# yj-yu/Recurrent_Gaze_Prediction

Measured on AMD Instinct MI355X. Metric: frames/sec (49x49 saliency maps), gaze_grcn 16-frame clips, higher is better.
Workload: dtype bf16; 1 GPU; gaze_grcn end-to-end: synthetic 16x112x112x3 windows -> C3D conv1a-5b -> 1024->512 proj -> ConvGRU(512->128, 7x7) -> deconv head -> 49x49 softmax maps; clips_per_gpu=64, n_lstm_steps=16, parallelism=dp1 (clip-sharded replicas, no collective), weights=random init (reference initialisers), GRU filters std 0.05

## Files before the change

include/rgp.h:

```cpp
#ifndef RGP_H_
#define RGP_H_
#include <stddef.h>

#ifdef __cplusplus
extern "C" {
#endif

#define RGP_OK 0
#define RGP_EINVAL (-1)
#define RGP_EHIP (-2)
#define RGP_EWORKSPACE (-3)
#define RGP_ESTATE (-4)
#define RGP_ETIMEOUT (-5)

#define RGP_F32 0
#define RGP_BF16 1

typedef void* rgp_stream_t;

const char* rgp_last_error(void);
int rgp_version(void);
int rgp_device_arch(char* buf, int buflen);

typedef struct rgp_grcn rgp_grcn_t;
// ... 204 lines not shown
int rgp_shallownet_forward(rgp_shallownet_t* plan, const float* frames, int n_frames, float* saliency,
                           float* saliency7, rgp_stream_t stream);

int rgp_shallownet_create_ex(rgp_shallownet_t** plan, int max_frames, int image_hw, int dtype, int save_for_backward);
int rgp_shallownet_backward(rgp_shallownet_t* plan, int n_frames, const float* d_saliency, const rgp_shallownet_weights* grads,
                            rgp_stream_t stream);

typedef struct rgp_cascade rgp_cascade_t;

typedef struct rgp_cascade_weights {
  const float *proj_c3d_W, *proj_c3d_b;
  const float *bottom_Wz, *bottom_Uz, *bottom_Wr, *bottom_Ur, *bottom_W, *bottom_U;
  const float* upsampling_weight;
  const float *top_Wz, *top_Uz, *top_Wr, *top_Ur, *top_W, *top_U;
  const float *fc1_w, *fc1_b, *fc2_w, *fc2_b;
  rgp_shallownet_weights shallownet;
} rgp_cascade_weights;

int rgp_cascade_create(rgp_cascade_t** plan, int batch, int n_steps, int image_hw, int dtype);
int rgp_cascade_destroy(rgp_cascade_t* plan);
size_t rgp_cascade_workspace_bytes(const rgp_cascade_t* plan);
int rgp_cascade_bind_workspace(rgp_cascade_t* plan, void* workspace, size_t bytes, rgp_stream_t stream);
int rgp_cascade_set_weights(rgp_cascade_t* plan, const rgp_cascade_weights* w, rgp_stream_t stream);
int rgp_cascade_forward(rgp_cascade_t* plan, const float* frame_images, const float* c3d_input, float* gazemaps,
                        rgp_stream_t stream);
int rgp_cascade_create_ex(rgp_cascade_t** plan, int batch, int n_steps, int image_hw, int dtype, int save_for_backward);
int rgp_cascade_backward(rgp_cascade_t* plan, const float* gazemaps, const float* gt_gazemap, const rgp_cascade_weights* grads,
                         float* d_rows, rgp_stream_t stream);
int rgp_cascade_set_dropout(rgp_cascade_t* plan, float keep_prob, const unsigned char* mask);
int rgp_cascade_read_buffer(rgp_cascade_t* plan, const char* name, float* dst, rgp_stream_t stream);

typedef struct rgp_c3d rgp_c3d_t;

typedef struct rgp_c3d_weights {
  const float* w[8];
  const float* b[8];
} rgp_c3d_weights;

int rgp_c3d_create(rgp_c3d_t** plan, int max_windows, int dtype);
int rgp_c3d_destroy(rgp_c3d_t* plan);
size_t rgp_c3d_workspace_bytes(const rgp_c3d_t* plan);
int rgp_c3d_bind_workspace(rgp_c3d_t* plan, void* workspace, size_t bytes, rgp_stream_t stream);
int rgp_c3d_set_weights(rgp_c3d_t* plan, const rgp_c3d_weights* w, rgp_stream_t stream);
int rgp_c3d_forward(rgp_c3d_t* plan, const float* video, int n_windows, float* features, void* rows,
                    rgp_stream_t stream);
int rgp_c3d_forward_frames(rgp_c3d_t* plan, const unsigned char* frames, int n_frames, int frame_h, int frame_w,
                           const int* window_starts, int n_windows, const float* mean_cube, float* features, void* rows,
                           rgp_stream_t stream);
int rgp_c3d_frames_to_video(rgp_c3d_t* plan, const unsigned char* frames, int n_frames, int frame_h, int frame_w,
                            const int* window_starts, int n_windows, const float* mean_cube, float* video,
                            rgp_stream_t stream);
int rgp_c3d_read_layer(rgp_c3d_t* plan, int layer, int n_windows, float* dst, rgp_stream_t stream);
size_t rgp_c3d_layer_elems(const rgp_c3d_t* plan, int layer, int n_windows);

int rgp_c3d_create_ex(rgp_c3d_t** plan, int max_windows, int dtype, int flags);
#define RGP_C3D_SAVE_FOR_BACKWARD 1
#define RGP_C3D_KERNELS_IGEMM 2
#define RGP_C3D_KERNELS_TILE128 4
#define RGP_C3D_CONV2A_ROWWISE 8
const char* rgp_c3d_layer_kernel_name(const rgp_c3d_t* plan, int layer, int n_windows);
size_t rgp_c3d_param_elems(const rgp_c3d_t* plan);
size_t rgp_c3d_param_offset(const rgp_c3d_t* plan, int layer, int is_bias);
int rgp_c3d_backward(rgp_c3d_t* plan, const float* d_features, const float* d_rows, int n_windows, float* grads,
                     rgp_stream_t stream);
int rgp_c3d_wait_layer_grads(rgp_c3d_t* plan, int layer, rgp_stream_t waiting_stream);
int rgp_c3d_read_grad_image(rgp_c3d_t* plan, int layer, int n_windows, float* dst, rgp_stream_t stream);

#define RGP_C3D_STAGES 9
int rgp_c3d_profile_enable(rgp_c3d_t* plan, int enable);
int rgp_c3d_profile_read(rgp_c3d_t* plan, double ms[RGP_C3D_STAGES], long long calls[RGP_C3D_STAGES]);

#define RGP_METRICS_MAX_PIX 4096
#define RGP_METRICS_MAX_FIX 256
#define RGP_METRICS_MAX_THRESHOLDS 1024
#define RGP_METRICS_COUNT 6
#define RGP_METRIC_SIM 1
#define RGP_METRIC_CC 2
#define RGP_METRIC_AUC_JUDD 4
#define RGP_METRIC_AUC_BORJI 8
#define RGP_METRIC_AUC_SHUFFLED 16
#define RGP_METRIC_NSS 32
#define RGP_METRIC_ALL 63
#define RGP_METRIC_ROW_SIM 0
#define RGP_METRIC_ROW_CC 1
#define RGP_METRIC_ROW_AUC_JUDD 2
#define RGP_METRIC_ROW_AUC_BORJI 3
#define RGP_METRIC_ROW_AUC_SHUFFLED 4
#define RGP_METRIC_ROW_NSS 5
#define RGP_METRICS_DEVICE_DRAWS 1
#define RGP_METRICS_NO_JITTER 2
#define RGP_METRICS_PRED_F64 4
#define RGP_METRICS_GT_F64 8

typedef struct rgp_metrics_args {
  const void* pred;
  const void* gt;
  const float* fix;
  const float* other;
  long long other_stride;
  int n_frames, height, width;
  unsigned metrics;
  unsigned flags;
  int n_rep;
  int neg_stride;
  double step_size;
  const double* judd_jitter;
// ... 65 lines not shown
```

recurrent_gaze_prediction_amd/_lib.py:

```python
import ctypes
import os

import torch

LIB_PATH = os.path.join(os.path.dirname(os.path.abspath(__file__)), 'librgp_hip.so')

RGP_F32, RGP_BF16 = 0, 1
RGP_ETIMEOUT = -5
RGP_GRCN_SAVE_FOR_BACKWARD, RGP_GRCN_PER_STEP, RGP_GRCN_UNFOLDED_HEAD = 1, 2, 4
RGP_C3D_SAVE_FOR_BACKWARD, RGP_C3D_KERNELS_IGEMM, RGP_C3D_KERNELS_TILE128, RGP_C3D_CONV2A_ROWWISE = 1, 2, 4, 8
RGP_C3DCONV_SAVE_FOR_BACKWARD, RGP_C3DCONV_STAGED, RGP_C3DCONV_FUSED = 1, 2, 4
RGP_LSTM_SAVE_FOR_BACKWARD, RGP_LSTM_PER_STEP, RGP_LSTM_PERSISTENT, RGP_LSTM_BPTT_PERSISTENT = 1, 2, 4, 8
RGP_GRCN77_SAVE_FOR_BACKWARD, RGP_GRCN77_PER_STEP = 1, 2
RGP_FAULT_SEQ_LOST_MEMBER, RGP_FAULT_BPTT_LOST_MEMBER = 1, 2
RGP_ACTION_NN, RGP_ACTION_SVM = 0, 1
RGP_ACTION_USE_GAZEMAP, RGP_ACTION_SAVE_FOR_BACKWARD, RGP_ACTION_UNFUSED = 1, 2, 4
RGP_GRCN_GRADS_TOP, RGP_GRCN_GRADS_GRU, RGP_GRCN_GRADS_PROJ = 0, 1, 2
RGP_SQNORM_PARTIALS = 256
RGP_METRICS_MAX_PIX, RGP_METRICS_MAX_FIX, RGP_METRICS_MAX_THRESHOLDS, RGP_METRICS_COUNT = 4096, 256, 1024, 6
METRIC_BITS = {'sim': 1, 'cc': 2, 'AUC_Judd': 4, 'AUC_Borji': 8, 'AUC_shuffled': 16, 'NSS': 32}
METRIC_ROWS = {'sim': 0, 'cc': 1, 'AUC_Judd': 2, 'AUC_Borji': 3, 'AUC_shuffled': 4, 'NSS': 5}
RGP_METRICS_DEVICE_DRAWS, RGP_METRICS_NO_JITTER, RGP_METRICS_PRED_F64, RGP_METRICS_GT_F64 = 1, 2, 4, 8
RGP_GTMAPS_MAX_PIX, RGP_GTMAPS_MAX_OBSERVERS, RGP_GTMAPS_MAX_RADIUS = 4096, 32, 32
DTYPES = {'f32': RGP_F32, 'fp32': RGP_F32, 'float32': RGP_F32, 'bf16': RGP_BF16, 'bfloat16': RGP_BF16}
# ... 133 lines not shown
    'rgp_lstm_bptt_persistent_workgroups': (c_int, [c_void_p]),
    'rgp_lstm_read_buffer': (c_int, [c_void_p, c_char_p, c_void_p, c_void_p]),
    'rgp_lstm_buffer_elems': (c_size_t, [c_void_p, c_char_p]),
    'rgp_grcn77_create': (c_int, [ctypes.POINTER(c_void_p), c_int, c_int, c_int, c_int]),
    'rgp_grcn77_destroy': (c_int, [c_void_p]),
    'rgp_grcn77_workspace_bytes': (c_size_t, [c_void_p]),
    'rgp_grcn77_bind_workspace': (c_int, [c_void_p, c_void_p, c_size_t, c_void_p]),
    'rgp_grcn77_set_weights': (c_int, [c_void_p, ctypes.POINTER(Grcn77Weights), c_void_p]),
    'rgp_grcn77_forward': (c_int, [c_void_p, c_void_p, c_void_p, c_void_p, c_void_p]),
    'rgp_grcn77_forward_rows': (c_int, [c_void_p, c_void_p, c_void_p, c_void_p, c_void_p]),
    'rgp_grcn77_state_elems': (c_size_t, [c_void_p]),
    'rgp_grcn77_forward_stream': (c_int, [c_void_p, c_void_p, c_void_p, c_void_p, c_void_p, c_int, c_void_p, c_void_p, c_void_p]),
    'rgp_grcn77_backward': (c_int, [c_void_p, c_void_p, c_void_p, c_void_p, ctypes.POINTER(Grcn77Weights), c_int, c_void_p]),
    'rgp_grcn77_backward_input': (c_int, [c_void_p, c_void_p, c_void_p]),
    'rgp_grcn77_status': (c_int, [c_void_p, c_void_p]),
    'rgp_grcn77_persistent_workgroups': (c_int, [c_void_p]),
    'rgp_grcn77_read_buffer': (c_int, [c_void_p, c_char_p, c_void_p, c_void_p]),
    'rgp_grcn77_buffer_elems': (c_size_t, [c_void_p, c_char_p]),
    'rgp_grcn77_head_fwd': (c_int, [c_void_p, c_void_p, c_void_p, c_void_p, c_void_p]),
    'rgp_shallownet_create_ex': (c_int, [ctypes.POINTER(c_void_p), c_int, c_int, c_int, c_int]),
    'rgp_shallownet_backward': (c_int, [c_void_p, c_int, c_void_p, ctypes.POINTER(ShallowNetWeights), c_void_p]),
    'rgp_shallownet_create': (c_int, [ctypes.POINTER(c_void_p), c_int, c_int, c_int]),
    'rgp_shallownet_destroy': (c_int, [c_void_p]),
    'rgp_shallownet_workspace_bytes': (c_size_t, [c_void_p]),
    'rgp_shallownet_bind_workspace': (c_int, [c_void_p, c_void_p, c_size_t, c_void_p]),
    'rgp_shallownet_set_weights': (c_int, [c_void_p, ctypes.POINTER(ShallowNetWeights), c_void_p]),
    'rgp_shallownet_forward': (c_int, [c_void_p, c_void_p, c_int, c_void_p, c_void_p, c_void_p]),
    'rgp_cascade_create': (c_int, [ctypes.POINTER(c_void_p), c_int, c_int, c_int, c_int]),
    'rgp_cascade_destroy': (c_int, [c_void_p]),
    'rgp_cascade_workspace_bytes': (c_size_t, [c_void_p]),
    'rgp_cascade_bind_workspace': (c_int, [c_void_p, c_void_p, c_size_t, c_void_p]),
    'rgp_cascade_set_weights': (c_int, [c_void_p, ctypes.POINTER(CascadeWeights), c_void_p]),
    'rgp_cascade_forward': (c_int, [c_void_p, c_void_p, c_void_p, c_void_p, c_void_p]),
    'rgp_cascade_read_buffer': (c_int, [c_void_p, c_char_p, c_void_p, c_void_p]),
    'rgp_cascade_create_ex': (c_int, [ctypes.POINTER(c_void_p), c_int, c_int, c_int, c_int, c_int]),
    'rgp_cascade_backward': (c_int, [c_void_p, c_void_p, c_void_p, ctypes.POINTER(CascadeWeights), c_void_p, c_void_p]),
    'rgp_c3d_create': (c_int, [ctypes.POINTER(c_void_p), c_int, c_int]),
    'rgp_c3d_destroy': (c_int, [c_void_p]),
    'rgp_c3d_workspace_bytes': (c_size_t, [c_void_p]),
    'rgp_c3d_bind_workspace': (c_int, [c_void_p, c_void_p, c_size_t, c_void_p]),
    'rgp_c3d_set_weights': (c_int, [c_void_p, ctypes.POINTER(C3DWeights), c_void_p]),
    'rgp_c3d_forward': (c_int, [c_void_p, c_void_p, c_int, c_void_p, c_void_p, c_void_p]),
    'rgp_c3d_forward_frames': (c_int, [c_void_p, c_void_p, c_int, c_int, c_int, ctypes.POINTER(c_int), c_int, c_void_p,
                                       c_void_p, c_void_p, c_void_p]),
    'rgp_c3d_frames_to_video': (c_int, [c_void_p, c_void_p, c_int, c_int, c_int, ctypes.POINTER(c_int), c_int, c_void_p,
                                        c_void_p, c_void_p]),
    'rgp_c3d_create_ex': (c_int, [ctypes.POINTER(c_void_p), c_int, c_int, c_int]),
    'rgp_c3d_param_elems': (c_size_t, [c_void_p]),
    'rgp_c3d_param_offset': (c_size_t, [c_void_p, c_int, c_int]),
    'rgp_c3d_backward': (c_int, [c_void_p, c_void_p, c_void_p, c_int, c_void_p, c_void_p]),
    'rgp_c3d_read_grad_image': (c_int, [c_void_p, c_int, c_int, c_void_p, c_void_p]),
    'rgp_c3d_read_layer': (c_int, [c_void_p, c_int, c_int, c_void_p, c_void_p]),
    'rgp_c3d_layer_elems': (c_size_t, [c_void_p, c_int, c_int]),
    'rgp_grcn_backward': (c_int, [c_void_p, c_void_p, c_void_p, c_void_p, ctypes.POINTER(GrcnWeights), c_int, c_void_p]),
    'rgp_adam_clip_step': (c_int, [c_void_p, c_void_p, c_void_p, c_void_p, ctypes.c_longlong, c_void_p, c_int,
                                   ctypes.c_float, ctypes.c_float, ctypes.c_float, ctypes.c_float, ctypes.c_float,
                                   c_void_p, c_void_p]),
    'rgp_global_sqnorm': (c_int, [c_void_p, ctypes.c_longlong, c_void_p, c_void_p]),
    'rgp_adam_clip_step_ext': (c_int, [c_void_p, c_void_p, c_void_p, c_void_p, ctypes.c_longlong, c_void_p, c_int, c_int,
                                       ctypes.c_float, ctypes.c_float, ctypes.c_float, ctypes.c_float, ctypes.c_float,
                                       c_void_p, c_void_p]),
    'rgp_lr_schedule_step': (c_int, [c_void_p, ctypes.c_float, ctypes.c_float, c_int, ctypes.c_float, ctypes.c_float,
                                     c_void_p, c_void_p]),
    'rgp_adam_clip_step_dev': (c_int, [c_void_p, c_void_p, c_void_p, c_void_p, ctypes.c_longlong, c_void_p, c_int, c_void_p,
                                       ctypes.c_float, ctypes.c_float, ctypes.c_float, ctypes.c_float, c_void_p, c_void_p]),
    'rgp_momentum_clip_step': (c_int, [c_void_p, c_void_p, c_void_p, ctypes.c_longlong, c_void_p, c_int, ctypes.c_float,
                                       ctypes.c_float, ctypes.c_float, c_void_p, c_void_p]),
    'rgp_rmsprop_clip_step': (c_int, [c_void_p, c_void_p, c_void_p, c_void_p, ctypes.c_longlong, c_void_p, c_int,
                                      ctypes.c_float, ctypes.c_float, ctypes.c_float, ctypes.c_float, ctypes.c_float,
                                      c_void_p, c_void_p]),
    'rgp_l2_loss_fwd': (c_int, [c_void_p, c_void_p, ctypes.c_longlong, c_int, c_void_p, c_void_p, c_void_p]),
    'rgp_dropout_mask': (c_int, [c_void_p, ctypes.c_longlong, ctypes.c_float, ctypes.c_ulonglong, ctypes.c_ulonglong, c_void_p]),
    'rgp_metrics_workspace_bytes': (c_size_t, [c_int, c_int, c_int, ctypes.c_uint]),
    'rgp_saliency_scores': (c_int, [ctypes.POINTER(MetricsArgs), c_void_p]),
    'rgp_metrics_status': (c_int, [c_void_p, c_void_p]),
    'rgp_gtmaps_workspace_bytes': (c_size_t, []),
    'rgp_gazemaps_from_fixations': (c_int, [ctypes.POINTER(GtmapsArgs), c_void_p]),
    'rgp_gtmaps_status': (c_int, [c_void_p, c_void_p]),
    'rgp_dropout_apply': (c_int, [c_void_p, c_void_p, ctypes.c_longlong, ctypes.c_float, c_void_p]),
    'rgp_fcgru_set_dropout': (c_int, [c_void_p, ctypes.c_float, c_void_p]),
    'rgp_cascade_set_dropout': (c_int, [c_void_p, ctypes.c_float, c_void_p]),
    'rgp_c3d_wait_layer_grads': (c_int, [c_void_p, c_int, c_void_p]),
    'rgp_grcn_wait_grads': (c_int, [c_void_p, c_int, c_void_p]),
    'rgp_grcn_grads_top_early': (c_int, [c_void_p]),
    'rgp_grcn_persistent_workgroups': (c_int, [c_void_p]),
    'rgp_grcn_profile_enable': (c_int, [c_void_p, c_int]),
    'rgp_grcn_profile_read': (c_int, [c_void_p, ctypes.POINTER(ctypes.c_double), ctypes.POINTER(ctypes.c_longlong)]),
    'rgp_c3d_profile_enable': (c_int, [c_void_p, c_int]),
    'rgp_c3d_profile_read': (c_int, [c_void_p, ctypes.POINTER(ctypes.c_double), ctypes.POINTER(ctypes.c_longlong)]),
    'rgp_action_create': (c_int, [ctypes.POINTER(c_void_p), c_int, c_int, c_int, c_int, c_int]),
    'rgp_action_destroy': (c_int, [c_void_p]),
    'rgp_action_workspace_bytes': (c_size_t, [c_void_p]),
    'rgp_action_bind_workspace': (c_int, [c_void_p, c_void_p, c_size_t, c_void_p]),
    'rgp_action_set_weights': (c_int, [c_void_p, ctypes.POINTER(ActionWeights), c_void_p]),
    'rgp_action_get_weights': (c_int, [c_void_p, ctypes.POINTER(ActionWeights), c_void_p]),
    'rgp_action_bind_slots': (c_int, [c_void_p, ctypes.POINTER(ActionWeights), ctypes.POINTER(ActionWeights)]),
    'rgp_action_forward': (c_int, [c_void_p, c_void_p, c_void_p, c_void_p, c_void_p, c_void_p]),
    'rgp_action_forward_rows': (c_int, [c_void_p, c_void_p, c_void_p, c_void_p, c_void_p, c_void_p]),
    'rgp_action_loss': (c_int, [c_void_p, c_void_p, c_void_p, c_void_p]),
    'rgp_action_train_step': (c_int, [c_void_p, c_void_p, c_void_p, c_void_p, c_int, ctypes.c_float, c_void_p, c_void_p]),
    'rgp_action_fc1_fwd': (c_int, [c_void_p, c_void_p, c_void_p, c_void_p]),
    'rgp_action_tail': (c_int, [c_void_p, c_void_p, c_void_p]),
    'rgp_action_fc1_update': (c_int, [c_void_p, c_void_p, c_void_p, c_void_p, c_int, ctypes.c_float, c_void_p]),
    'rgp_action_read_buffer': (c_int, [c_void_p, c_char_p, c_void_p, c_void_p]),
    'rgp_action_buffer_elems': (c_size_t, [c_void_p, c_char_p]),
}
# ... 50 lines not shown
```

recurrent_gaze_prediction_amd/csrc/conv1a.hip.h:

```cpp
#pragma once
#include "igemm.hip.h"

namespace rgp {

struct Conv1aParams {
  const float* video;
  const bf16_t* in;
  const bf16_t* wp;
  const float* bias;
  bf16_t* out;
  unsigned char* argmax;
  int n_windows;
};

constexpr int C1_D = 16, C1_H = 112, C1_HP = 114, C1_WP = 116, C1_K = 128;
constexpr int C1_KSTEPS = 7;
constexpr int C1_PO = 56;
constexpr int C1_XG = C1_PO / 8;
constexpr int C1_OUT_P = 58;
constexpr int C1_JROWS = 4;
constexpr int C1_YQ = C1_PO / C1_JROWS;
constexpr int C1_PROWS = 2 * C1_JROWS + 2;
constexpr int C1_ROWB = C1_WP * 8;
constexpr int C1_WPL = 144;
constexpr int C1_SLAB = C1_PROWS * C1_WPL * 8;
constexpr int C1_SMEM = 4 * C1_SLAB;
constexpr int C1_STREAM = C1_D + 2;
constexpr int C1_CPR = C1_WP * 8 / 16;
constexpr int C1_CHUNKS = C1_PROWS * C1_CPR;
constexpr int C1_NLD = (C1_CHUNKS + 255) / 256;
constexpr int C1F_GROUPS = C1_PROWS * 28;
constexpr int C1F_NLD = (C1F_GROUPS + 255) / 256;

template <int V> struct C1Int { static constexpr int value = V; };
typedef unsigned u32x2 __attribute__((ext_vector_type(2)));
typedef short s16x8_c1 __attribute__((ext_vector_type(8)));
typedef float f32x16 __attribute__((ext_vector_type(16)));

template <int OFF>
static __device__ __forceinline__ u32x2 c1_lds_read64(unsigned addr) {
  u32x2 v;
  asm volatile("ds_read_b64 %0, %1 offset:%2" : "=v"(v) : "v"(addr), "n"(OFF));
  return v;
}
static __device__ __forceinline__ void c1_lds_wait(u32x2 (&a)[C1_KSTEPS][2]) {
  asm volatile("s_waitcnt lgkmcnt(0)"
               : "+v"(a[0][0]), "+v"(a[0][1]), "+v"(a[1][0]), "+v"(a[1][1]), "+v"(a[2][0]), "+v"(a[2][1]), "+v"(a[3][0]),
                 "+v"(a[3][1]), "+v"(a[4][0]), "+v"(a[4][1]), "+v"(a[5][0]), "+v"(a[5][1]), "+v"(a[6][0]), "+v"(a[6][1]));
}
static constexpr __host__ __device__ int c1_tap_kz(int tap) { return (tap > 26 ? 13 : tap) / 9; }

template <bool FUSED, bool ARGMAX, int VAR = 0>
static __global__ __launch_bounds__(256, 2) void conv1a_pool_bf16_kernel(const Conv1aParams p) {
  constexpr int WPL = C1_WPL;
  constexpr int XS = FUSED ? 1 : 0;
  extern __shared__ __attribute__((aligned(16))) char c1_smem[];
  char* ring = c1_smem;
  for (int i = threadIdx.x; i < C1_SMEM / 16; i += 256) ((u32x4*)ring)[i] = (u32x4){0u, 0u, 0u, 0u};
  __syncthreads();
  const int tid = threadIdx.x;
  const int lane = tid & 63;
  const int wave = __builtin_amdgcn_readfirstlane(tid >> 6);
  const int frow = lane & 31, kh = lane >> 5;

  const long long total = (long long)p.n_windows * C1_YQ;
  const long long per_xcd = (total + 7) / 8;
  const int xcd = blockIdx.x & 7, slot = blockIdx.x >> 3, nslot = gridDim.x >> 3;
  long long col = xcd * per_xcd + slot;
  long long col_end = (xcd + 1) * per_xcd;
  if (col_end > total) col_end = total;
  if (col >= col_end) return;

  u32x4 bfrag[C1_KSTEPS][2];
#pragma unroll
  for (int s = 0; s < C1_KSTEPS; ++s)
#pragma unroll
    for (int nt = 0; nt < 2; ++nt)
      bfrag[s][nt] = *(const u32x4*)(p.wp + (frow * 2 + nt) * C1_K + s * 16 + kh * 8);
#pragma unroll
  for (int nt = 0; nt < 2; ++nt) {
    const float b = p.bias[frow * 2 + nt];
    const bf16_t hi = f2bf(b);
    const bf16_t lo = f2bf(b - bf2f(hi));
    if (kh == 0) bfrag[3][nt][3] = (bfrag[3][nt][3] & 0xffffu) | ((unsigned)hi << 16);
    else bfrag[6][nt][3] = (bfrag[6][nt][3] & 0xffffu) | ((unsigned)lo << 16);
  }

  int g_off[C1_NLD], l_off[C1_NLD];
#pragma unroll
  for (int u = 0; u < C1_NLD; ++u) {
    int q = tid + 256 * u;
    if (q >= C1_CHUNKS) q = C1_CHUNKS - 1;
    const int ry = q / C1_CPR, c = q - ry * C1_CPR;
    g_off[u] = (ry * C1_WP) * 4 + c * 8;
    l_off[u] = ry * (WPL * 8) + c * 16;
  }
  auto fetch = [&](long long c, int pz, u32x4 (&pf)[C1_NLD]) {
    const int yq = (int)(c % C1_YQ);
    const long long n = c / C1_YQ;
    const bf16_t* src = p.in + (((n * (C1_D + 2) + pz) * C1_HP + yq * 2 * C1_JROWS) * (long long)C1_WP) * 4;
#pragma unroll
    for (int u = 0; u < C1_NLD; ++u) pf[u] = *(const u32x4*)(src + g_off[u]);
  };
  auto park = [&](char* slab, const u32x4 (&pf)[C1_NLD]) {
#pragma unroll
    for (int u = 0; u < C1_NLD; ++u)
      if (tid + 256 * u < C1_CHUNKS) {
        u32x4 v = pf[u];
        v[1] |= 0x3f800000u;
        v[3] |= 0x3f800000u;
        *(u32x4*)(slab + l_off[u]) = v;
      }
  };
  constexpr unsigned WIN_BYTES = C1_D * C1_H * C1_H * 12u;
  unsigned f_src[C1F_NLD], f_dst[C1F_NLD], f_edge = 0;
#pragma unroll
  for (int u = 0; u < C1F_NLD; ++u) {
    int q = tid + 256 * u;
    if (q >= C1F_GROUPS) q = C1F_GROUPS - 1;
    const int ry = q / 28, xg = q - ry * 28;
    f_src[u] = (unsigned)((ry * C1_H + 4 * xg) * 12);
    f_dst[u] = (unsigned)((ry * WPL + 2 + 4 * xg) * 8);
    if (ry == 0) f_edge |= 1u << u;
    if (ry == C1_PROWS - 1) f_edge |= 16u << u;
  }
  auto fetch_f = [&](long long c, int pz, f32x4 (&pf)[C1F_NLD][3]) {
    const int yq = (int)(c % C1_YQ);
    const long long n = c / C1_YQ;
    const auto rsrc = __builtin_amdgcn_make_buffer_rsrc(const_cast<float*>(p.video + n * (long long)(WIN_BYTES / 4)), 0,
                                                        WIN_BYTES, 0x00020000);
    const bool plane_ok = pz >= 1 && pz <= C1_D;
    const unsigned job_off = (unsigned)((((pz - 1) * C1_H + yq * 2 * C1_JROWS - 1) * C1_H) * 12);
    const unsigned edge = plane_ok ? f_edge & ((yq == 0 ? 0xfu : 0u) | (yq == C1_YQ - 1 ? 0xf0u : 0u)) : 0xffu;
#pragma unroll
    for (int u = 0; u < C1F_NLD; ++u) {
      const unsigned off = (edge & (0x11u << u)) ? 0x80000000u : f_src[u] + job_off;
#pragma unroll
      for (int k = 0; k < 3; ++k)
        pf[u][k] = __builtin_bit_cast(f32x4, __builtin_amdgcn_raw_buffer_load_b128(rsrc, off + 16 * k, 0, 0));
    }
  };
  typedef float f32x2_t __attribute__((ext_vector_type(2)));
  typedef __bf16 bf16x2_t __attribute__((ext_vector_type(2)));
  auto pk = [](float x, float y) -> unsigned {
    const f32x2_t v = {x, y};
    return __builtin_bit_cast(unsigned, __builtin_convertvector(v, bf16x2_t));
  };
  auto park_f = [&](char* slab, const f32x4 (&pf)[C1F_NLD][3]) {
#pragma unroll
    for (int u = 0; u < C1F_NLD; ++u) {
      if (tid + 256 * u < C1F_GROUPS) {
        const float f[12] = {pf[u][0][0], pf[u][0][1], pf[u][0][2], pf[u][0][3], pf[u][1][0], pf[u][1][1],
                             pf[u][1][2], pf[u][1][3], pf[u][2][0], pf[u][2][1], pf[u][2][2], pf[u][2][3]};
        u32x4 w0, w1;
#pragma unroll
        for (int px = 0; px < 4; ++px) {
          const unsigned lo = pk(f[3 * px], f[3 * px + 1]), hi = pk(f[3 * px + 2], 1.f);
          if (px < 2) { w0[2 * px] = lo; w0[2 * px + 1] = hi; } else { w1[2 * (px - 2)] = lo; w1[2 * (px - 2) + 1] = hi; }
        }
        char* dst = slab + f_dst[u];
        *(u32x4*)dst = w0;
        *(u32x4*)(dst + 16) = w1;
      }
    }
  };

  const int r_w = frow >> 2, r_dy = (frow >> 1) & 1, r_dx = frow & 1;
  const unsigned lds0 = (unsigned)(size_t)(__attribute__((address_space(3))) char*)c1_smem;
  const unsigned lane_base = lds0 + ((r_dy + 2 * wave) * WPL + 2 * r_w + r_dx + XS) * 8;
  unsigned ra0[C1_KSTEPS][2];
#pragma unroll
  for (int s = 0; s < C1_KSTEPS; ++s)
#pragma unroll
    for (int j = 0; j < 2; ++j) {
      int tap = 4 * s + 2 * kh + j;
      if (tap > 26) tap = 13;
      const int ky = (tap / 3) % 3, kx = tap % 3;
      ra0[s][j] = (ky * WPL + kx) * 8 + lane_base;
    }

  auto load_frags = [&](auto OFF, const unsigned (&ra)[C1_KSTEPS][2], u32x2 (&a)[C1_KSTEPS][2]) {
    constexpr int off = decltype(OFF)::value;
#pragma unroll
    for (int s = 0; s < C1_KSTEPS; ++s)
#pragma unroll
      for (int j = 0; j < 2; ++j) a[s][j] = c1_lds_read64<off>(ra[s][j]);
  };
  const int o_lane = kh * 64 + frow * 2;
  auto tile = [&](bf16_t* orow, unsigned char* arow, int xg, const u32x2 (&a)[C1_KSTEPS][2]) {
    f32x16 acc[2];
#pragma unroll
    for (int nt = 0; nt < 2; ++nt)
#pragma unroll
      for (int i = 0; i < 16; ++i) acc[nt][i] = 0.f;
#pragma unroll
    for (int s = 0; s < C1_KSTEPS; ++s) {
      const u32x4 av = {a[s][0][0], a[s][0][1], a[s][1][0], a[s][1][1]};
#pragma unroll
      for (int nt = 0; nt < 2; ++nt)
        acc[nt] = __builtin_amdgcn_mfma_f32_32x32x16_bf16(__builtin_bit_cast(s16x8_c1, av),
                                                          __builtin_bit_cast(s16x8_c1, bfrag[s][nt]), acc[nt], 0, 0, 0);
    }
    unsigned dpk[4];
#pragma unroll
// ... 18 lines not shown
        if ((dpk[j] & 0x7fffu) == 0) codes |= 4u;
        if ((dpk[j] & 0x7fff0000u) == 0) codes |= 4u << 8;
        *(unsigned short*)(arow + (xg * 8 + 2 * j) * 64 + o_lane) = (unsigned short)codes;
      }
    }
    if (!(VAR & 2) || p.n_windows < 0) {
      const bool odd = (frow & 1) != 0;
#pragma unroll
      for (int pp = 0; pp < 2; ++pp) {
        const unsigned send = odd ? dpk[2 * pp] : dpk[2 * pp + 1];
        const unsigned recv = (unsigned)__builtin_amdgcn_mov_dpp((int)send, 0xB1, 0xF, 0xF, true);
        uint2 o;
        o.x = odd ? recv : dpk[2 * pp];
        o.y = odd ? dpk[2 * pp + 1] : recv;
        *(uint2*)(orow + (xg * 8 + 2 * (2 * pp + (odd ? 1 : 0))) * 64 + kh * 64 + (frow & ~1) * 2) = o;
      }
    }
  };
  auto compute = [&](long long c, int z, int rb) {
    const unsigned so[3] = {(unsigned)(rb & 3) * C1_SLAB, (unsigned)((rb + 1) & 3) * C1_SLAB, (unsigned)((rb + 2) & 3) * C1_SLAB};
    unsigned ra[C1_KSTEPS][2];
#pragma unroll
    for (int s = 0; s < C1_KSTEPS; ++s)
#pragma unroll
      for (int j = 0; j < 2; ++j) ra[s][j] = ra0[s][j] + (kh ? so[c1_tap_kz(4 * s + 2 + j)] : so[c1_tap_kz(4 * s + j)]);
    const int yo = (int)(c % C1_YQ) * C1_JROWS + wave;
    const long long n = c / C1_YQ;
    bf16_t* orow = p.out + (((n * (C1_D + 2) + z + 1) * C1_OUT_P + yo + 1) * (long long)C1_OUT_P + 1) * 64;
    unsigned char* arow = ARGMAX ? p.argmax + (((n * C1_D + z) * C1_PO + yo) * (long long)C1_PO) * 64 : nullptr;
    u32x2 a0[C1_KSTEPS][2], a1[C1_KSTEPS][2];
    load_frags(C1Int<0>{}, ra, a0);
    c1_lds_wait(a0);
    load_frags(C1Int<128>{}, ra, a1);
    tile(orow, arow, 0, a0);
    c1_lds_wait(a1);
    load_frags(C1Int<256>{}, ra, a0);
    tile(orow, arow, 1, a1);
    c1_lds_wait(a0);
    load_frags(C1Int<384>{}, ra, a1);
    tile(orow, arow, 2, a0);
    c1_lds_wait(a1);
    load_frags(C1Int<512>{}, ra, a0);
    tile(orow, arow, 3, a1);
    c1_lds_wait(a0);
    load_frags(C1Int<640>{}, ra, a1);
    tile(orow, arow, 4, a0);
    c1_lds_wait(a1);
    load_frags(C1Int<768>{}, ra, a0);
    tile(orow, arow, 5, a1);
    c1_lds_wait(a0);
    tile(orow, arow, 6, a0);
  };

  u32x4 pf[C1_NLD];
  f32x4 pff[C1F_NLD][3];
  int pz = 0, i = 0;
  if constexpr (FUSED) { fetch_f(col, 0, pff); park_f(ring, pff); }
  else { fetch(col, 0, pf); park(ring, pf); }
  __syncthreads();
  while (true) {
    const bool wrap = pz == C1_STREAM - 1;
    const long long ncol = wrap ? col + nslot : col;
    const int npz = wrap ? 0 : pz + 1;
    const bool more = ncol < col_end;
    if (more && (!(VAR & 4) || i < 4)) { if constexpr (FUSED) fetch_f(ncol, npz, pff); else fetch(ncol, npz, pf); }
    if (pz >= 2) compute(col, pz - 2, i - 2);
    if (!more) break;
    char* slab = ring + ((i + 1) & 3) * C1_SLAB;
    if constexpr (FUSED) park_f(slab, pff); else park(slab, pf);
    __syncthreads();
    ++i;
    col = ncol;
    pz = npz;
  }
}

}
```

recurrent_gaze_prediction_amd/csrc/rgp_c3d.hip:

```cpp
#include <algorithm>

#include "rgp_c3d_plan.h"
#include "conv1a.hip.h"

using namespace rgp;

namespace {

template <typename T, int G, int P>
int run_layer(rgp_c3d* c, int i, int n, hipStream_t s) {
  IgemmParams p = make_params(c->L[i], c->ws + c->act_off[i], c->ws, n);
  p.tile128 = c->tile128();
  EpiParams e = make_epi(c->L[i], c->ws + c->act_off[i + 1], c->ws);
  e.bias = c->bias[i];
  if (c->save && P > 1) e.argmax = (unsigned char*)(c->ws + c->B[i].argmax_off);
#ifdef RGP_DEV_KNOBS
  const int stamp_layer = dev_knob("RGP_STAMP", -1);
  if (stamp_layer == i) {
    static unsigned long long* dbg = nullptr;
    const int nblk = (p.M + 255) / 256 * ((p.N + 127) / 128);
    if (!dbg) RGP_HIP(hipMalloc(&dbg, (size_t)nblk * 64 * 8));
    RGP_HIP(hipMemsetAsync(dbg, 0, (size_t)nblk * 64 * 8, s));
    e.c_save = (float*)dbg;
    const int rc = launch_igemm<T, G, P, EpiStore<T, true, true>>(p, e, s);
// ... 264 lines not shown
        frames, frame_h, frame_w, (const int*)(c->ws + c->starts_off), mean_cube, nullptr,
        video + (size_t)w0 * 16 * 112 * 112 * 3, npix);
    RGP_HIP(hipGetLastError());
  }
  return RGP_OK;
}

const char* rgp_c3d_layer_kernel_name(const rgp_c3d_t* c, int i, int n_windows) {
  static thread_local char buf[96];
  buf[0] = 0;
  if (!c || i < 0 || i > 7 || n_windows <= 0) return buf;
  const int n = std::min(n_windows, c->max_windows);
  const C3dLayerSpec& l = kLayers[i];
  const int P = l.pd * l.ph * l.ph;
  const bool bf = c->dtype == RGP_BF16;
  if (bf && i == 0) {
    snprintf(buf, sizeof(buf), "conv1a_pool_bf16_kernel<%s>", c->save ? "act0,argmax" : "fused");
  } else if (bf && c->use_patch() && i >= 1 && i <= 3 && (i == 1 || c->L[i].chunk_major == 64)) {
    snprintf(buf, sizeof(buf), "conv_patch%s_bf16_kernel<%d,%d,%d,%d,pool%d>", i == 1 && c->conv2a_slab() ? "_slab" : "", l.cin, l.cout,
             l.H, l.D, P);
  } else if (bf && c->use_patch() && (i == 4 || i == 5) && c->L[i].chunk_major == 64) {
    snprintf(buf, sizeof(buf), "conv_patch14_bf16_kernel<%d,pool%d>", l.cin, P);
  } else if (bf && c->use_patch() && (i == 6 || i == 7) && c->L[i].chunk_major == 64) {
    snprintf(buf, sizeof(buf), "conv_patch7_bf16_kernel<%s>", i == 6 ? "image" : "rows");
  } else {
    IgemmParams p = make_params(c->L[i], c->ws, c->ws, n);
    p.tile128 = c->tile128();
    IgemmTile t;
    using EB = EpiStore<bf16_t, true, true>;
    using EF = EpiStore<float, true, true>;
    if (bf) t = P == 8 ? igemm_tile_choice<bf16_t, 1, 8, EB>(p, 1) : P == 4 ? igemm_tile_choice<bf16_t, 4, 4, EB>(p, 1) : igemm_tile_choice<bf16_t, 1, 1, EB>(p, 1);
    else t = P == 8 ? igemm_tile_choice<float, 1, 8, EF>(p, 1) : P == 4 ? igemm_tile_choice<float, 2, 4, EF>(p, 1) : igemm_tile_choice<float, 1, 1, EF>(p, 1);
    snprintf(buf, sizeof(buf), "%s,%s,pool%d>", igemm_tile_name(t), bf ? "bf16" : "f32", P);
  }
  return buf;
}

int rgp_c3d_profile_enable(rgp_c3d_t* c, int enable) {
  RGP_REQUIRE(c, "rgp_c3d_profile_enable: null plan");
  c->prof.enabled = enable != 0;
  return RGP_OK;
}

int rgp_c3d_profile_read(rgp_c3d_t* c, double ms[RGP_C3D_STAGES], long long calls[RGP_C3D_STAGES]) {
  RGP_REQUIRE(c && ms && calls, "rgp_c3d_profile_read: null argument");
  return c->prof.read(ms, calls, RGP_C3D_STAGES);
}

size_t rgp_c3d_layer_elems(const rgp_c3d_t* c, int layer, int n_windows) {
  if (!c || layer < 0 || layer > 7) return 0;
  return (size_t)n_windows * c->unpad_tab[layer].size() * kLayers[layer].cout;
}

int rgp_c3d_read_layer(rgp_c3d_t* c, int layer, int n_windows, float* dst, rgp_stream_t stream) {
  RGP_REQUIRE(c && c->ws && dst && layer >= 0 && layer <= 7 && n_windows > 0 && n_windows <= c->max_windows,
              "rgp_c3d_read_layer: bad arguments");
  hipStream_t s = (hipStream_t)stream;
  const int rows = (int)c->unpad_tab[layer].size();
  int C = kLayers[layer].cout;
  const long long stride = c->L[layer].out_img_stride;
  if (layer == 7) {
  }
  const long long total = (long long)n_windows * rows * C;
  const int blocks = (int)std::min<long long>((total + 255) / 256, 8192);
  const int* tab = (const int*)(c->ws + c->unpad_off[layer]);
  const char* src = c->ws + c->act_off[layer + 1];
  if (c->dtype == RGP_BF16) unpad_kernel<bf16_t><<<blocks, 256, 0, s>>>((const bf16_t*)src, dst, tab, rows, C, stride, total);
  else unpad_kernel<float><<<blocks, 256, 0, s>>>((const float*)src, dst, tab, rows, C, stride, total);
  RGP_HIP(hipGetLastError());
  return RGP_OK;
}

}
```

recurrent_gaze_prediction_amd/csrc/rgp_conv1a.hip:

```cpp
#include "rgp_c3d_plan.h"
#include "conv1a.hip.h"

using namespace rgp;

int run_conv1a_bf16(rgp_c3d* c, int n, hipStream_t s, const float* video) {
  Conv1aParams p;
  p.video = video;
  p.in = (const bf16_t*)(c->ws + c->act_off[0]);
  p.wp = (const bf16_t*)(c->ws + c->L[0].w_off);
  p.bias = c->bias[0];
  p.out = (bf16_t*)(c->ws + c->act_off[1]);
  p.argmax = c->save ? (unsigned char*)(c->ws + c->B[0].argmax_off) : nullptr;
  p.n_windows = n;
  int n_cu = 0;
  RGP_TRY(device_cu_count(&n_cu));
  const int grid = 2 * n_cu;
  auto launch = [&](auto kern) -> int {
    RGP_TRY(ensure_dyn_smem((const void*)kern, C1_SMEM));
    kern<<<grid, 256, C1_SMEM, s>>>(p);
    RGP_HIP(hipGetLastError());
    return RGP_OK;
  };
#ifdef RGP_DEV_KNOBS
  if (video && !p.argmax) switch (dev_knob("RGP_C1VAR", 0)) {
    case 2: return launch(conv1a_pool_bf16_kernel<true, false, 2>);
    case 4: return launch(conv1a_pool_bf16_kernel<true, false, 4>);
    case 6: return launch(conv1a_pool_bf16_kernel<true, false, 6>);
    default: break;
  }
#endif
  if (video && !p.argmax) return launch(conv1a_pool_bf16_kernel<true, false>);
  if (video) return launch(conv1a_pool_bf16_kernel<true, true>);
  if (p.argmax) return launch(conv1a_pool_bf16_kernel<false, true>);
  return launch(conv1a_pool_bf16_kernel<false, false>);
}
```

recurrent_gaze_prediction_amd/engine.py:

```python
import ctypes

import numpy as np
import torch

from . import _lib

GRCN_PARAM_TO_FIELD = {
    'proj_c3d_W': 'proj_c3d_W', 'proj_c3d_b': 'proj_c3d_b',
    'GRU_Conv_Wz': 'gru_Wz', 'GRU_Conv_Uz': 'gru_Uz', 'GRU_Conv_Wr': 'gru_Wr', 'GRU_Conv_Ur': 'gru_Ur',
    'GRU_Conv_W': 'gru_W', 'GRU_Conv_U': 'gru_U', 'bn_gamma': 'bn_gamma', 'bn_beta': 'bn_beta',
    'weight1': 'up_weight1', 'weight2': 'up_weight2', 'weight3': 'up_weight3', 'out_W': 'out_W', 'out_b': 'out_b',
}
C3D_LAYER_NAMES = ('conv1a', 'conv2a', 'conv3a', 'conv3b', 'conv4a', 'conv4b', 'conv5a', 'conv5b')
C3D_EXTENTS = ((16, 112), (16, 56), (8, 28), (8, 28), (4, 14), (4, 14), (2, 7), (2, 7))
C3D_CHANNELS = ((3, 64), (64, 128), (128, 256), (256, 256), (256, 512), (512, 512), (512, 512), (512, 512))


def _stream_ptr(device):
    return ctypes.c_void_p(torch.cuda.current_stream(device).cuda_stream)


def _ptr(t):
    return ctypes.c_void_p(t.data_ptr()) if t is not None else None

# ... 809 lines not shown
        return self.flat_grads[ow:ow + 27 * cin * cout + cout]

    def wait_layer_grads(self, layer, stream):
        _lib.check(self.lib.rgp_c3d_wait_layer_grads(self._h, int(layer), ctypes.c_void_p(stream.cuda_stream)))

    def read_grad_image(self, layer, n_windows):
        d, h = C3D_EXTENTS[layer]
        out = torch.empty(n_windows, d, h, h, C3D_CHANNELS[layer][1], device=self.device)
        with torch.cuda.device(self.device):
            _lib.check(self.lib.rgp_c3d_read_grad_image(self._h, layer, n_windows, _ptr(out), _stream_ptr(self.device)))
        return out

    def _frames_args(self, frames, window_starts, mean_cube):
        assert frames.is_cuda and frames.dtype == torch.uint8 and frames.is_contiguous() and frames.dim() == 4
        assert frames.shape[3] == 3, tuple(frames.shape)
        starts = [int(v) for v in window_starts]
        arr = (ctypes.c_int * len(starts))(*starts)
        if mean_cube is not None:
            assert mean_cube.is_cuda and mean_cube.dtype == torch.float32 and mean_cube.is_contiguous()
            assert tuple(mean_cube.shape) == (3, 16, 128, 171), tuple(mean_cube.shape)
        return arr, len(starts)

    def forward_frames(self, frames, window_starts, mean_cube=None, want_features=True, want_rows=False, out_rows=None):
        arr, n = self._frames_args(frames, window_starts, mean_cube)
        feats = torch.empty(n, 1024, 7, 7, device=self.device) if want_features else None
        rows = out_rows
        if want_rows and rows is None:
            rows = torch.empty(n * 49, 1024, dtype=self.torch_dtype, device=self.device)
        with torch.cuda.device(self.device):
            _lib.check(self.lib.rgp_c3d_forward_frames(self._h, _ptr(frames), frames.shape[0], frames.shape[1],
                                                       frames.shape[2], arr, n, _ptr(mean_cube), _ptr(feats), _ptr(rows),
                                                       _stream_ptr(self.device)))
        return feats, rows

    def frames_to_video(self, frames, window_starts, mean_cube=None):
        arr, n = self._frames_args(frames, window_starts, mean_cube)
        video = torch.empty(n, 16, 112, 112, 3, device=self.device)
        with torch.cuda.device(self.device):
            _lib.check(self.lib.rgp_c3d_frames_to_video(self._h, _ptr(frames), frames.shape[0], frames.shape[1],
                                                        frames.shape[2], arr, n, _ptr(mean_cube), _ptr(video),
                                                        _stream_ptr(self.device)))
        return video

    def layer_kernel_name(self, layer, n_windows):
        return self.lib.rgp_c3d_layer_kernel_name(self._h, int(layer), int(n_windows)).decode()

    def read_layer(self, layer, n_windows):
        n = self.lib.rgp_c3d_layer_elems(self._h, layer, n_windows)
        out = torch.empty(n, dtype=torch.float32, device=self.device)
        with torch.cuda.device(self.device):
            _lib.check(self.lib.rgp_c3d_read_layer(self._h, layer, n_windows, _ptr(out), _stream_ptr(self.device)))
        return out

    def profile(self, enable=True):
        _lib.check(self.lib.rgp_c3d_profile_enable(self._h, int(enable)))

    def profile_read(self):
        n = len(_lib.C3D_STAGES)
        ms, calls = (ctypes.c_double * n)(), (ctypes.c_longlong * n)()
        _lib.check(self.lib.rgp_c3d_profile_read(self._h, ms, calls))
        return {k: (ms[i], calls[i]) for i, k in enumerate(_lib.C3D_STAGES)}


ACTION_PARAM_TO_FIELD = {
    'NN': {'W1': 'W1', 'Wg': 'Wg', 'b1': 'b1', 'W2': 'W2', 'b2': 'b2', 'W3': 'W3', 'b3': 'b3'},
    'SVM': {'W1': 'W1', 'Wg': 'Wg', 'b1': 'b1'},
}


def action_learning_rate(step, lr0=0.002, decay=0.96, decay_steps=10):
    return float(lr0) * float(decay) ** (float(step) / float(decay_steps))


class ActionEngine(object):

    def __init__(self, batch, dim_feat=1024, mode='NN', use_gazemap=False, dtype='bf16', save_for_backward=False,
                 device='cuda:0', unfused=False):
        self.lib = _lib.load()
        self.device = _require_gpu(device)
        self.B, self.C, self.K = int(batch), int(dim_feat), 49 * int(dim_feat)
        self.mode, self.use_gazemap, self.dtype = mode, bool(use_gazemap), dtype
        self.N = 256 if mode == 'NN' else 13
        self.save_for_backward, self.unfused = bool(save_for_backward), bool(unfused)
        self.torch_dtype = torch.bfloat16 if _lib.DTYPES[dtype] == _lib.RGP_BF16 else torch.float32
        self.names = tuple(k for k in ACTION_PARAM_TO_FIELD[mode] if k != 'Wg' or self.use_gazemap)
        self.flat_params = self.weights = self.adam_m = self.adam_v = None
        flags = (_lib.RGP_ACTION_USE_GAZEMAP if use_gazemap else 0) | (_lib.RGP_ACTION_SAVE_FOR_BACKWARD if save_for_backward else 0) \
            | (_lib.RGP_ACTION_UNFUSED if unfused else 0)
        self._f = {k[len('rgp_action_'):]: getattr(self.lib, k) for k in _lib.SIGNATURES if k.startswith('rgp_action_')}
        self._h = ctypes.c_void_p()
        with torch.cuda.device(self.device):
            _lib.check(self._f['create'](ctypes.byref(self._h), self.B, self.C, {'NN': _lib.RGP_ACTION_NN, 'SVM': _lib.RGP_ACTION_SVM}[mode],
                                         _lib.DTYPES[dtype], flags))
            nbytes = self._f['workspace_bytes'](self._h)
            self.workspace = torch.empty(nbytes, dtype=torch.uint8, device=self.device)
            _lib.check(self._f['bind_workspace'](self._h, _ptr(self.workspace), nbytes, _stream_ptr(self.device)))

    def __del__(self):
        h, self._h = getattr(self, '_h', None), None
        if h:
            self._f['destroy'](h)

    def _st(self, views):
        return _struct(_lib.ActionWeights, {k: ACTION_PARAM_TO_FIELD[self.mode][k] for k in self.names}, views)

    def shapes(self):
# ... 110 lines not shown
```

Measured before the change: 21480 frames/s.

## Add dedicated producer waves to conv1a fused kernel for load/compute overlap

Result: no change. 21370 frames/s (-0.5%).

```diff
diff --git a/include/rgp.h b/include/rgp.h
--- a/include/rgp.h
+++ b/include/rgp.h
@@ -280,6 +280,7 @@
                             rgp_stream_t stream);
 int rgp_c3d_read_layer(rgp_c3d_t* plan, int layer, int n_windows, float* dst, rgp_stream_t stream);
 size_t rgp_c3d_layer_elems(const rgp_c3d_t* plan, int layer, int n_windows);
+size_t rgp_c3d_layer_image_offset(const rgp_c3d_t* plan, int layer, int padded_dims[4]);
 
 int rgp_c3d_create_ex(rgp_c3d_t** plan, int max_windows, int dtype, int flags);
 #define RGP_C3D_SAVE_FOR_BACKWARD 1
diff --git a/recurrent_gaze_prediction_amd/_lib.py b/recurrent_gaze_prediction_amd/_lib.py
--- a/recurrent_gaze_prediction_amd/_lib.py
+++ b/recurrent_gaze_prediction_amd/_lib.py
@@ -209,6 +209,7 @@
     'rgp_c3d_read_grad_image': (c_int, [c_void_p, c_int, c_int, c_void_p, c_void_p]),
     'rgp_c3d_read_layer': (c_int, [c_void_p, c_int, c_int, c_void_p, c_void_p]),
     'rgp_c3d_layer_elems': (c_size_t, [c_void_p, c_int, c_int]),
+    'rgp_c3d_layer_image_offset': (c_size_t, [c_void_p, c_int, c_void_p]),
     'rgp_grcn_backward': (c_int, [c_void_p, c_void_p, c_void_p, c_void_p, ctypes.POINTER(GrcnWeights), c_int, c_void_p]),
     'rgp_adam_clip_step': (c_int, [c_void_p, c_void_p, c_void_p, c_void_p, ctypes.c_longlong, c_void_p, c_int,
                                    ctypes.c_float, ctypes.c_float, ctypes.c_float, ctypes.c_float, ctypes.c_float,
diff --git a/recurrent_gaze_prediction_amd/csrc/conv1a.hip.h b/recurrent_gaze_prediction_amd/csrc/conv1a.hip.h
--- a/recurrent_gaze_prediction_amd/csrc/conv1a.hip.h
+++ b/recurrent_gaze_prediction_amd/csrc/conv1a.hip.h
@@ -49,14 +49,18 @@
                  "+v"(a[3][1]), "+v"(a[4][0]), "+v"(a[4][1]), "+v"(a[5][0]), "+v"(a[5][1]), "+v"(a[6][0]), "+v"(a[6][1]));
 }
 static constexpr __host__ __device__ int c1_tap_kz(int tap) { return (tap > 26 ? 13 : tap) / 9; }
-
-template <bool FUSED, bool ARGMAX, int VAR = 0>
-static __global__ __launch_bounds__(256, 2) void conv1a_pool_bf16_kernel(const Conv1aParams p) {
+static __device__ __forceinline__ void c1_job_barrier() { asm volatile("s_barrier" ::: "memory"); }
+static __device__ __forceinline__ void c1_job_barrier_parked() { asm volatile("s_waitcnt lgkmcnt(0)\n\ts_barrier" ::: "memory"); }
+
+template <bool FUSED, bool ARGMAX, int NPROD = 0, int VAR = 0>
+static __global__ __launch_bounds__(256 + 64 * NPROD, 2) void conv1a_pool_bf16_kernel(const Conv1aParams p) {
+  static_assert(NPROD == 0 || (FUSED && !ARGMAX && NPROD <= 2), "producer waves: the fused inference instance only");
+  constexpr int NT = 256 + 64 * NPROD;
   constexpr int WPL = C1_WPL;
   constexpr int XS = FUSED ? 1 : 0;
   extern __shared__ __attribute__((aligned(16))) char c1_smem[];
   char* ring = c1_smem;
-  for (int i = threadIdx.x; i < C1_SMEM / 16; i += 256) ((u32x4*)ring)[i] = (u32x4){0u, 0u, 0u, 0u};
+  for (int i = threadIdx.x; i < C1_SMEM / 16; i += NT) ((u32x4*)ring)[i] = (u32x4){0u, 0u, 0u, 0u};
   __syncthreads();
   const int tid = threadIdx.x;
   const int lane = tid & 63;
@@ -113,28 +117,34 @@
       }
   };
   constexpr unsigned WIN_BYTES = C1_D * C1_H * C1_H * 12u;
-  unsigned f_src[C1F_NLD], f_dst[C1F_NLD], f_edge = 0;
-#pragma unroll
-  for (int u = 0; u < C1F_NLD; ++u) {
-    int q = tid + 256 * u;
-    if (q >= C1F_GROUPS) q = C1F_GROUPS - 1;
-    const int ry = q / 28, xg = q - ry * 28;
+  constexpr int FT = NPROD ? 64 * NPROD : 256;
+  constexpr int FNLD = (C1F_GROUPS + FT - 1) / FT;
+  const int ftid = NPROD ? tid - 256 : tid;
+  unsigned f_src[FNLD], f_dst[FNLD], f_edge = 0;
+#pragma unroll
+  for (int u = 0; u < FNLD; ++u) {
+    int q = ftid + FT * u;
+    const bool none = q >= C1F_GROUPS;
+    if (none) q = C1F_GROUPS - 1;
+    int ry = q / 28, xg = q - ry * 28;
+    if (NPROD > 0 && none) { xg = 29; f_edge |= 0x10000u << u; }
     f_src[u] = (unsigned)((ry * C1_H + 4 * xg) * 12);
     f_dst[u] = (unsigned)((ry * WPL + 2 + 4 * xg) * 8);
     if (ry == 0) f_edge |= 1u << u;
-    if (ry == C1_PROWS - 1) f_edge |= 16u << u;
+    if (ry == C1_PROWS - 1) f_edge |= 0x100u << u;
   }
-  auto fetch_f = [&](long long c, int pz, f32x4 (&pf)[C1F_NLD][3]) {
+  auto fetch_f = [&](long long c, int pz, f32x4 (&pf)[FNLD][3]) {
     const int yq = (int)(c % C1_YQ);
     const long long n = c / C1_YQ;
     const auto rsrc = __builtin_amdgcn_make_buffer_rsrc(const_cast<float*>(p.video + n * (long long)(WIN_BYTES / 4)), 0,
                                                         WIN_BYTES, 0x00020000);
     const bool plane_ok = pz >= 1 && pz <= C1_D;
     const unsigned job_off = (unsigned)((((pz - 1) * C1_H + yq * 2 * C1_JROWS - 1) * C1_H) * 12);
-    const unsigned edge = plane_ok ? f_edge & ((yq == 0 ? 0xfu : 0u) | (yq == C1_YQ - 1 ? 0xf0u : 0u)) : 0xffu;
-#pragma unroll
-    for (int u = 0; u < C1F_NLD; ++u) {
-      const unsigned off = (edge & (0x11u << u)) ? 0x80000000u : f_src[u] + job_off;
+    unsigned edge = plane_ok ? f_edge & ((yq == 0 ? 0xffu : 0u) | (yq == C1_YQ - 1 ? 0xff00u : 0u)) : 0xffffu;
+    if constexpr (NPROD > 0) edge |= f_edge & 0xff0000u;
+#pragma unroll
+    for (int u = 0; u < FNLD; ++u) {
+      const unsigned off = (edge & (0x10101u << u)) ? 0x80000000u : f_src[u] + job_off;
 #pragma unroll
       for (int k = 0; k < 3; ++k)
         pf[u][k] = __builtin_bit_cast(f32x4, __builtin_amdgcn_raw_buffer_load_b128(rsrc, off + 16 * k, 0, 0));
@@ -146,10 +156,10 @@
     const f32x2_t v = {x, y};
     return __builtin_bit_cast(unsigned, __builtin_convertvector(v, bf16x2_t));
   };
-  auto park_f = [&](char* slab, const f32x4 (&pf)[C1F_NLD][3]) {
-#pragma unroll
-    for (int u = 0; u < C1F_NLD; ++u) {
-      if (tid + 256 * u < C1F_GROUPS) {
+  auto park_f = [&](char* slab, const f32x4 (&pf)[FNLD][3]) {
+#pragma unroll
+    for (int u = 0; u < FNLD; ++u) {
+      if (NPROD > 0 || ftid + FT * u < C1F_GROUPS) {
         const float f[12] = {pf[u][0][0], pf[u][0][1], pf[u][0][2], pf[u][0][3], pf[u][1][0], pf[u][1][1],
                              pf[u][1][2], pf[u][1][3], pf[u][2][0], pf[u][2][1], pf[u][2][2], pf[u][2][3]};
         u32x4 w0, w1;
@@ -274,26 +284,60 @@
     tile(orow, arow, 6, a0);
   };
 
-  u32x4 pf[C1_NLD];
-  f32x4 pff[C1F_NLD][3];
   int pz = 0, i = 0;
-  if constexpr (FUSED) { fetch_f(col, 0, pff); park_f(ring, pff); }
-  else { fetch(col, 0, pf); park(ring, pf); }
-  __syncthreads();
-  while (true) {
-    const bool wrap = pz == C1_STREAM - 1;
-    const long long ncol = wrap ? col + nslot : col;
-    const int npz = wrap ? 0 : pz + 1;
-    const bool more = ncol < col_end;
-    if (more && (!(VAR & 4) || i < 4)) { if constexpr (FUSED) fetch_f(ncol, npz, pff); else fetch(ncol, npz, pf); }
-    if (pz >= 2) compute(col, pz - 2, i - 2);
-    if (!more) break;
-    char* slab = ring + ((i + 1) & 3) * C1_SLAB;
-    if constexpr (FUSED) park_f(slab, pff); else park(slab, pf);
+  if constexpr (NPROD > 0) {
+    if (wave >= 4) {
+      f32x4 pff[FNLD][3];
+      fetch_f(col, 0, pff);
+      park_f(ring, pff);
+      c1_job_barrier_parked();
+      while (true) {
+        const bool wrap = pz == C1_STREAM - 1;
+        const long long ncol = wrap ? col + nslot : col;
+        const int npz = wrap ? 0 : pz + 1;
+        if (!(ncol < col_end)) break;
+        if (!(VAR & 4) || i < 4) fetch_f(ncol, npz, pff);
+        park_f(ring + ((i + 1) & 3) * C1_SLAB, pff);
+        c1_job_barrier_parked();
+        ++i;
+        col = ncol;
+        pz = npz;
+      }
+    } else {
+      c1_job_barrier();
+      while (true) {
+        const bool wrap = pz == C1_STREAM - 1;
+        const long long ncol = wrap ? col + nslot : col;
+        const int npz = wrap ? 0 : pz + 1;
+        if (pz >= 2) compute(col, pz - 2, i - 2);
+        if (!(ncol < col_end)) break;
+        c1_job_barrier();
+        ++i;
+        col = ncol;
+        pz = npz;
+      }
+    }
+  } else {
+    u32x4 pf[C1_NLD];
+    f32x4 pff[FNLD][3];
+    if constexpr (FUSED) { fetch_f(col, 0, pff); park_f(ring, pff); }
+    else { fetch(col, 0, pf); park(ring, pf); }
     __syncthreads();
-    ++i;
-    col = ncol;
-    pz = npz;
+    while (true) {
+      const bool wrap = pz == C1_STREAM - 1;
+      const long long ncol = wrap ? col + nslot : col;
+      const int npz = wrap ? 0 : pz + 1;
+      const bool more = ncol < col_end;
+      if (more && (!(VAR & 4) || i < 4)) { if constexpr (FUSED) fetch_f(ncol, npz, pff); else fetch(ncol, npz, pf); }
+      if (pz >= 2) compute(col, pz - 2, i - 2);
+      if (!more) break;
+      char* slab = ring + ((i + 1) & 3) * C1_SLAB;
+      if constexpr (FUSED) park_f(slab, pff); else park(slab, pf);
+      __syncthreads();
+      ++i;
+      col = ncol;
+      pz = npz;
+    }
   }
 }
 
diff --git a/recurrent_gaze_prediction_amd/csrc/rgp_c3d.hip b/recurrent_gaze_prediction_amd/csrc/rgp_c3d.hip
--- a/recurrent_gaze_prediction_amd/csrc/rgp_c3d.hip
+++ b/recurrent_gaze_prediction_amd/csrc/rgp_c3d.hip
@@ -340,6 +340,17 @@
   return (size_t)n_windows * c->unpad_tab[layer].size() * kLayers[layer].cout;
 }
 
+size_t rgp_c3d_layer_image_offset(const rgp_c3d_t* c, int layer, int padded_dims[4]) {
+  if (!c || layer < 0 || layer > 6) return 0;
+  const C3dLayerSpec& l = kLayers[layer];
+  if (padded_dims) {
+    padded_dims[0] = l.D / l.pd + 2;
+    padded_dims[1] = padded_dims[2] = l.H / l.ph + 2;
+    padded_dims[3] = l.cout;
+  }
+  return c->act_off[layer + 1];
+}
+
 int rgp_c3d_read_layer(rgp_c3d_t* c, int layer, int n_windows, float* dst, rgp_stream_t stream) {
   RGP_REQUIRE(c && c->ws && dst && layer >= 0 && layer <= 7 && n_windows > 0 && n_windows <= c->max_windows,
               "rgp_c3d_read_layer: bad arguments");
diff --git a/recurrent_gaze_prediction_amd/csrc/rgp_conv1a.hip b/recurrent_gaze_prediction_amd/csrc/rgp_conv1a.hip
--- a/recurrent_gaze_prediction_amd/csrc/rgp_conv1a.hip
+++ b/recurrent_gaze_prediction_amd/csrc/rgp_conv1a.hip
@@ -15,21 +15,28 @@
   int n_cu = 0;
   RGP_TRY(device_cu_count(&n_cu));
   const int grid = 2 * n_cu;
-  auto launch = [&](auto kern) -> int {
+  auto launch = [&](auto kern, int nprod = 0) -> int {
     RGP_TRY(ensure_dyn_smem((const void*)kern, C1_SMEM));
-    kern<<<grid, 256, C1_SMEM, s>>>(p);
+    kern<<<grid, 256 + 64 * nprod, C1_SMEM, s>>>(p);
     RGP_HIP(hipGetLastError());
     return RGP_OK;
   };
 #ifdef RGP_DEV_KNOBS
-  if (video && !p.argmax) switch (dev_knob("RGP_C1VAR", 0)) {
-    case 2: return launch(conv1a_pool_bf16_kernel<true, false, 2>);
-    case 4: return launch(conv1a_pool_bf16_kernel<true, false, 4>);
-    case 6: return launch(conv1a_pool_bf16_kernel<true, false, 6>);
-    default: break;
+  if (video && !p.argmax) {
+    switch (dev_knob("RGP_C1VAR", 0)) {
+      case 2: return launch(conv1a_pool_bf16_kernel<true, false, 1, 2>, 1);
+      case 4: return launch(conv1a_pool_bf16_kernel<true, false, 1, 4>, 1);
+      case 6: return launch(conv1a_pool_bf16_kernel<true, false, 1, 6>, 1);
+      default: break;
+    }
+    switch (dev_knob("RGP_C1PROD", 1)) {
+      case 0: return launch(conv1a_pool_bf16_kernel<true, false, 0>);
+      case 2: return launch(conv1a_pool_bf16_kernel<true, false, 2>, 2);
+      default: break;
+    }
   }
 #endif
-  if (video && !p.argmax) return launch(conv1a_pool_bf16_kernel<true, false>);
+  if (video && !p.argmax) return launch(conv1a_pool_bf16_kernel<true, false, 1>, 1);
   if (video) return launch(conv1a_pool_bf16_kernel<true, true>);
   if (p.argmax) return launch(conv1a_pool_bf16_kernel<false, true>);
   return launch(conv1a_pool_bf16_kernel<false, false>);
diff --git a/recurrent_gaze_prediction_amd/engine.py b/recurrent_gaze_prediction_amd/engine.py
--- a/recurrent_gaze_prediction_amd/engine.py
+++ b/recurrent_gaze_prediction_amd/engine.py
@@ -885,6 +885,16 @@
             _lib.check(self.lib.rgp_c3d_read_layer(self._h, layer, n_windows, _ptr(out), _stream_ptr(self.device)))
         return out
 
+    def layer_image(self, layer, n_windows):
+        dims = (ctypes.c_int * 4)()
+        off = self.lib.rgp_c3d_layer_image_offset(self._h, int(layer), dims)
+        assert off > 0 and 0 < n_windows <= self.max_windows, (layer, n_windows)
+        shape = (int(n_windows),) + tuple(dims)
+        nbytes = self.torch_dtype.itemsize
+        for d in shape:
+            nbytes *= d
+        return self.workspace[off:off + nbytes].view(self.torch_dtype).view(shape)
+
     def profile(self, enable=True):
         _lib.check(self.lib.rgp_c3d_profile_enable(self._h, int(enable)))
 
```
